# fegennari/3DWorld

Hardware: AMD Instinct MI355X
Metric: heightmap Gcells/sec (noise+erosion), 16384^2 grid (higher is better)
Workload: dtype f32

## Files before the change

### 3dworld_amd/csrc/terra_driver.hpp

```cpp
#pragma once
#include "terra_common.hpp"
#include "terra_noise.hpp"
#include "terra_erosion.hpp"
#include "terra_landscape.hpp"
#include "terra_modmap.hpp"
#include "terra_treemap.hpp"
#include "terra_treeplace.hpp"
#include "terra_decidplace.hpp"
#include "terra_sceneryplace.hpp"
#include "terra_flowers.hpp"
#include "terra_grassview.hpp"
#include "terra_treeao.hpp"
#include "terra_treeedit.hpp"
#include "terra_stage.hpp"
#include "../../include/terra.h"
#include <vector>
#include <map>
#include <string>
#include <algorithm>
#include <cmath>
#include <stdexcept>
#include <string.h>
#include <stdio.h>
#include <stdlib.h>

namespace terra {

struct sine_k_t {float xmdx[F_TABLE_SIZE], xconst[F_TABLE_SIZE], ymdy[F_TABLE_SIZE], yconst[F_TABLE_SIZE], yscale[F_TABLE_SIZE];};

struct grid_job_t {
	float mx0, my0, mdx, mdy;
	uint32_t nx, ny, nxp, nyp;
	int mode, shape, kstart, glaciate, use_sine_mag;
	float sine_offset;
	int plain_only;
	int fused = 0;
	float fast_amax = 0.0f;
	uint32_t row0 = 0;
	uint32_t ty0 = 0, tyn = 0;
};
TERRA_HD uint32_t job_window_first(grid_job_t const &job) {return job.tyn ? job.ty0*128u : 0u;}
TERRA_HD uint32_t job_window_end(grid_job_t const &job) {uint64_t const e = ((uint64_t)job.ty0 + job.tyn)*128u; return (job.tyn && e < job.ny) ? (uint32_t)e : job.ny;}
constexpr uint32_t SG_TURN_ROWS = 2048;
struct noise_turn_t {void *wait_for = nullptr, *record = nullptr; uint32_t rows = 0;};

constexpr unsigned VOX_SINES = 60, VOX_PARAMS = 7;

inline uint32_t round_up(uint32_t v, uint32_t m) {return (v + m - 1)/m*m;}

struct tile_ref_pod_t {int32_t tx, ty; uint32_t xi, yi;};
struct tile_band_t {uint32_t twx, twy, ostride, xsplit, xgap, ysplit, ygap;};
TERRA_HD uint32_t tile_band_coord(uint32_t c, uint32_t split, uint32_t gap) {return c + ((c >= split) ? gap : 0u);}

TERRA_HD float sine_cell(grid_job_t const &job, float const *xt, float const *yt, unsigned x, unsigned y) {
	float z = 0.0f;
	for (int k = job.kstart; k < F_TABLE_SIZE; ++k) {z += xt[(size_t)k*job.nxp + x]*yt[(size_t)k*job.nyp + y];}
	return z;
}
TERRA_HD float finish_cell(float z, grid_job_t const &job, noise_consts_t const &nc, sin_lut_t const &L, float const *smx, float const *smy, unsigned x, unsigned y) {
	if (job.mode == MGEN_SINE) {z = apply_noise_shape_final(z, job.shape, nc.hp);}
	if (job.glaciate) {
		float const xg = ((float)x*job.mdx + job.mx0)*nc.DX_VAL_INV, yg = ((float)(y + job.row0)*job.mdy + job.my0)*nc.DY_VAL_INV;
		z = glaciate_epilogue(z, job.use_sine_mag ? smx[x] : 0.0f, job.use_sine_mag ? smy[y] : 0.0f, job.sine_offset, xg, yg, nc, L);
	}
	return z;
}
TERRA_HD float sine_cell_fused(grid_job_t const &job, float const *xt, float const *yt, unsigned x, unsigned y) {
	float z = 0.0f;
	for (int k = job.kstart; k < F_TABLE_SIZE; ++k) {z = fmaf(xt[(size_t)k*job.nxp + x], yt[(size_t)k*job.nyp + y], z);}
	return z;
}
TERRA_HD float finish_cell_fused(float z, grid_job_t const &job, noise_consts_t const &nc, float const *smx, float const *smy, unsigned x, unsigned y) {
	if (job.glaciate) {
		if (nc.glaciate) {float const relh = (z + nc.zmax_est)*nc.zmax_est2_inv; z = fmaf((relh*relh)*relh, nc.zmax_est2, -nc.zmax_est);}
		if (job.use_sine_mag) {z = z + fmaf(smx[x], smy[y], job.sine_offset);}
	}
	return z;
}
TERRA_HD float noise_cell(grid_job_t const &job, noise_consts_t const &nc, unsigned x, unsigned y) {
	float const xval = ((float)x*job.mdx + job.mx0)*nc.DX_VAL_INV, yval = ((float)(y + job.row0)*job.mdy + job.my0)*nc.DY_VAL_INV;
	switch (job.mode) {
	case MGEN_PERLIN:      return noise_zval<MGEN_PERLIN>(xval, yval, job.shape, nc);
	case MGEN_DWARP_GPU:   return noise_zval<MGEN_DWARP_GPU>(xval, yval, job.shape, nc);
	case MGEN_SIMPLEX_GPU: return noise_zval<MGEN_SIMPLEX_GPU>(xval, yval, job.shape, nc);
	default:               return noise_zval<MGEN_SIMPLEX>(xval, yval, job.shape, nc);
	}
}


struct shadow_consts_t {
	float X_SCENE_SIZE, Y_SCENE_SIZE, DX_VAL, DY_VAL, DX_VAL_INV, DY_VAL_INV, zmin, zmax, dist, dirx, diry, dirz;
	int xsize, ysize;
	uint32_t mask_fill;
	TERRA_HD int xpos(float xval) const {return (int)((double)((xval + X_SCENE_SIZE)*DX_VAL_INV) + 0.5);}
	TERRA_HD int ypos(float yval) const {return (int)((double)((yval + Y_SCENE_SIZE)*DY_VAL_INV) + 0.5);}
	TERRA_HD float xval(int xp) const {return -X_SCENE_SIZE + DX_VAL*(float)xp;}
	TERRA_HD float yval(int yp) const {return -Y_SCENE_SIZE + DY_VAL*(float)yp;}
// ... 676 lines not shown
			sk.yscale[k] = mesh_scale_z_inv*sinTable[k][0];
			sk.xconst[k] = ms2*sinTable[k][4] + sinTable[k][2] + x_mult*mx0;
			sk.yconst[k] = ms2*sinTable[k][3] + sinTable[k][1] + y_mult*my0;
			sk.xmdx[k] = x_mult*dx; sk.ymdy[k] = y_mult*dy;
		}
		return sk;
	}

	bool sine_plain_only(int shp, int kstart) const {
		if (shp != 0 || hp.crack_lo < hp.crack_hi || (hp.volcano_width > 0.0f && hp.volcano_height > 0.0f) || consts().custom_glaciate_exp != 0.0f) return false;
		double bound = 0.0;
		for (int k = kstart; k < F_TABLE_SIZE; ++k) {bound += std::fabs((double)(mesh_scale_z_inv*sinTable[k][0]));}
		return (double)min_std(hp.plat_bot, hp.crat_h) > bound*1.001 + 1e-3;
	}

	void gen_grid_dev(float x0, float y0, float dx, float dy, uint32_t nx, uint32_t ny, uint32_t flags, int min_start_sin, float *d_out, float *h_minmax = nullptr, uint32_t row0 = 0, uint32_t nrows = 0xFFFFFFFFu, float *d_minmax = nullptr, noise_turn_t const *turn = nullptr) {
		require_scene();
		if (nx == 0 || ny == 0) throw std::invalid_argument("build_arrays: nx, ny must be > 0");
		if (nrows == 0xFFFFFFFFu) {if (row0 != 0) throw std::invalid_argument("gen_grid rows: row0 without a row count"); nrows = ny;}
		if (nrows == 0 || row0 >= ny || nrows > ny - row0) throw std::invalid_argument("gen_grid rows: [row0, row0 + nrows) must be a non-empty range inside the grid");
		grid_job_t job;
		job.mx0 = dx*x0; job.my0 = dy*y0; job.mdx = dx; job.mdy = dy; job.nx = nx; job.ny = nrows; job.row0 = row0; ny = nrows;
		job.nxp = round_up(nx, 128); job.nyp = round_up(ny, 128);
		bool const force_sine = (flags & TERRA_GEN_FORCE_SINE) != 0;
		job.mode = force_sine ? (int)MGEN_SINE : mode; job.shape = force_sine ? 0 : shape;
		job.kstart = imax(start_eval_sin, min_start_sin);
		job.glaciate = (flags & TERRA_GEN_GLACIATE) ? 1 : 0;
		job.use_sine_mag = (job.glaciate && hp.sine_mag > 0.0f) ? 1 : 0;
		job.sine_offset = hp.sine_bias*mesh_scale_z_inv;
		job.plain_only = (job.mode == MGEN_SINE && sine_plain_only(job.shape, job.kstart)) ? 1 : 0;
		job.fused = (((flags & (TERRA_GEN_FUSED | TERRA_GEN_FAST)) || opt.gen_fused) && fused_kernel_exists(job.mode, job.plain_only != 0)) ? (((flags & TERRA_GEN_FAST) || opt.gen_fused == 2) ? 2 : 1) : 0;
		job.fast_amax = sine_amp_max(job.kstart);
		noise_consts_t const nc = consts();
		sin_lut_t const L = lut();
		float *smx = scratch<float>(s_smx, job.nxp), *smy = scratch<float>(s_smy, job.nyp);
		uint32_t *d_mm = nullptr;
		bool const sine = (job.mode == MGEN_SINE);
		if (turn && turn->wait_for) {BE::event_synchronize(turn->wait_for);}
		if (h_minmax || d_minmax || sine) {d_mm = scratch<uint32_t>(s_mm, 2); if (!sine) {be.fill32(d_mm, 0xFFFFFFFFu, 2);}}
		bool fused;
		bool const sm_on = job.use_sine_mag != 0;
		float const sm_scale = hp.sine_mag*mesh_scale_z_inv, sm_freq = mesh_scale*hp.sine_freq, dxi = DX_VAL_INV, dyi = DY_VAL_INV;
		if (sm_on && job.mode != MGEN_SINE) {
			float const mx0 = job.mx0, my0 = job.my0, mdx = dx, mdy = dy;
			uint32_t const nxp = job.nxp, nyp = job.nyp;
			be.launch((size_t)nxp + nyp, [=] TERRA_LAMBDA (size_t i) {
				if (i < nxp) {smx[i] = (i < nx) ? sm_scale*L.COSF(((float)(unsigned)i*mdx + mx0)*dxi*sm_freq) : 0.0f;}
				else {unsigned const y = (unsigned)(i - nxp); smy[y] = (y < ny) ? L.COSF(((float)(y + row0)*mdy + my0)*dyi*sm_freq) : 0.0f;}
			});
		}
		if (job.mode == MGEN_SINE) {
			float const *st = sinTable_dev();
			float const msx = mesh_scale*DX_VAL_INV, msy = mesh_scale*DY_VAL_INV, ms2 = (float)(0.5*(double)mesh_scale), mszi = mesh_scale_z_inv, jmx0 = job.mx0, jmy0 = job.my0, mdx = dx, mdy = dy;
			float *xt = scratch<float>(s_xt, (size_t)F_TABLE_SIZE*job.nxp), *yt = scratch<float>(s_yt, (size_t)F_TABLE_SIZE*job.nyp);
			uint32_t const nxp = job.nxp, nyp = job.nyp;
			size_t const ntab = (size_t)F_TABLE_SIZE*(nxp + nyp);
			uint32_t *const mmz = d_mm;
			be.launch(ntab + (sm_on ? (size_t)nxp + nyp : 0), [=] TERRA_LAMBDA (size_t i) {
				if (i == 0) {mmz[0] = 0xFFFFFFFFu; mmz[1] = 0xFFFFFFFFu;}
				if (i < (size_t)F_TABLE_SIZE*nxp) {
					unsigned const k = (unsigned)(i / nxp), x = (unsigned)(i % nxp);
					float const *stk = st + 5*k;
					float const x_mult = msx*stk[4], xconst = ms2*stk[4] + stk[2] + x_mult*jmx0, xmdx = x_mult*mdx;
					xt[i] = (x < nx) ? L.SINF(xmdx*(float)x + xconst) : 0.0f;
				}
				else if (i < ntab) {
					size_t const j = i - (size_t)F_TABLE_SIZE*nxp;
					unsigned const k = (unsigned)(j / nyp), y = (unsigned)(j % nyp);
					float const *stk = st + 5*k;
					float const y_mult = msy*stk[3], yscale = mszi*stk[0], yconst = ms2*stk[3] + stk[1] + y_mult*jmy0, ymdy = y_mult*mdy;
					yt[j] = (y < ny) ? yscale*L.SINF(ymdy*(float)(y + row0) + yconst) : 0.0f;
				}
				else {
					size_t const q = i - ntab;
					if (q < nxp) {smx[q] = (q < nx) ? sm_scale*L.COSF(((float)(unsigned)q*mdx + jmx0)*dxi*sm_freq) : 0.0f;}
					else {unsigned const y = (unsigned)(q - nxp); smy[y] = (y < ny) ? L.COSF(((float)(y + row0)*mdy + jmy0)*dyi*sm_freq) : 0.0f;}
				}
			});
			uint32_t *const mm_arg = (h_minmax || d_minmax) ? d_mm : nullptr;
			uint32_t const nty = (ny + 127u)/128u, tail = (turn && turn->record && !job.fused) ? std::min((turn->rows + 127u)/128u, nty) : 0u;
			if (tail > 0 && tail < nty) {
				grid_job_t part = job;
				part.ty0 = 0; part.tyn = nty - tail;
				fused = be.sine_grid(part, nc, L, xt, yt, smx, smy, d_out, mm_arg);
				be.event_record(turn->record);
				part.ty0 = nty - tail; part.tyn = tail;
				be.sine_grid(part, nc, L, xt, yt, smx, smy, d_out, mm_arg);
			}
			else {
				fused = be.sine_grid(job, nc, L, xt, yt, smx, smy, d_out, mm_arg);
				if (turn && turn->record) {be.event_record(turn->record);}
			}
		}
		else {
			fused = be.noise_grid(job, nc, L, smx, smy, d_out, (h_minmax || d_minmax) ? d_mm : nullptr, d_noise_lut);
			if (turn && turn->record) {be.event_record(turn->record);}
		}
		if ((h_minmax || d_minmax) && !fused) {be.minmax(d_out, (size_t)nx*ny, d_mm);}
		if (d_minmax) {uint32_t const *mm = d_mm; be.launch(1, [=] TERRA_LAMBDA (size_t) {d_minmax[0] = ord2f(mm[0]); d_minmax[1] = ord2f(~mm[1]);}, 64);}
		if (h_minmax) {
			uint32_t out[2];
			be.d2h(out, d_mm, sizeof(out));
			h_minmax[0] = ord2f(out[0]); h_minmax[1] = ord2f(~out[1]);
		}
	}

	float eval_mesh_sin_terms(float xv, float yv) const {
		require_scene();
		sin_lut_t const HL = host_lut();
		float zval = 0.0f;
		for (int k = start_eval_sin; k < F_TABLE_SIZE; ++k) {
			float const *stk = sinTable[k];
			zval += stk[0]*HL.SINF(stk[3]*yv + stk[1])*HL.SINF(stk[4]*xv + stk[2]);
		}
		return zval;
	}
	void eval_points_dev(float const *d_xy, uint32_t n, uint32_t kind, float xy_scale, int no_xyoff, int xoff2, int yoff2, float *d_out) {
		require_scene();
		if (n == 0) return;
		if (kind > 1) throw std::invalid_argument("eval_points: kind must be TERRA_POINTS_SCALED or TERRA_POINTS_EXACT");
		noise_consts_t const nc = consts();
		sin_lut_t const L = lut();
		float const *st = sinTable_dev();
		hmap_view_t const hv = hmap_view();
		bool const hm = using_hmap(), hm_detail = using_hmap_with_detail();
		int const md = mode, shp = shape, k0 = start_eval_sin;
// ... 530 lines not shown
		report.window_shifts = hc.n_shift;
		report.critical_steps = hc.crit_steps; report.critical_shifts = hc.crit_shifts;
		report.clk_wave = hc.clk_wave; report.clk_init = hc.clk_init; report.clk_shift = hc.clk_shift; report.clk_tail = hc.clk_tail; report.clk_critical = hc.clk_crit;
		report.clk_shift_flush = hc.clk_sh_flush; report.clk_shift_prep = hc.clk_sh_prep; report.clk_shift_load = hc.clk_sh_load;
		report.crit_clk_flush = hc.crit_own_flush; report.crit_clk_load = hc.crit_own_load; report.crit_clk_prep = hc.crit_own_prep;
		report.crit_clk_shift = hc.crit_own_shift; report.crit_clk_edge = hc.crit_own_edge; report.crit_steps_own = hc.crit_own_steps;
		if (!record_touched) return false;
		uint32_t const ntouched = hc.touched;
		if (ntouched > sb.touched_cap) return false;
		uint32_t const *tch = sb.touched; float const mz = ec.min_zval; grid_view_t const gg = g;
		be.launch(ntouched, [=] TERRA_LAMBDA (size_t i) {touched_clamp_body(gg, tch, (uint32_t)i, d_min ? *d_min : mz);});
		return true;
	}

	uint32_t tile_size() const {return (uint32_t)cfg.mesh_x;}
	void require_tile_size() const {
		int const S = cfg.mesh_x;
		if (S == 128) return;
		if (S < 16 || S > 1024) throw std::invalid_argument("tiles: the tile size (mesh_x) must be 16 .. 1024");
		if (cfg.mesh_y != S) throw std::invalid_argument("tiles: at a tile size other than 128 mesh_x and mesh_y must be equal (the reference asserts it in tiled mode)");
		if ((S & 3) == 2) throw std::invalid_argument("tiles: a tile size of the form 4k + 2 is not supported (the reference's sub-block loop would read row and column S + 2, past the zvals)");
	}
	void require_tile_128(char const *what) const {
		if (cfg.mesh_x != 128) throw std::invalid_argument(std::string(what) + ": only at the tile size 128 (mesh_x = 128)");
	}
	tile_ref_pod_t const *tile_fields_dev(int32_t const *tile_xy, uint32_t n, uint32_t tw, int shift, float *d_out, float xy_scale = 1.0f,
		bool glac = true, bool force_sine = false, int min_start_sin = 0,
		tile_band_t const *band = nullptr, bool *band_used = nullptr,
		float y_scale = 0.0f)
	{
		uint32_t const size = tile_size(), zv = tw;
		if (band_used) {*band_used = false;}
		float const fdx = xy_scale*DX_VAL, fdy = ((y_scale != 0.0f) ? y_scale : xy_scale)*DY_VAL;
		std::vector<int32_t> ux, uy;
		for (uint32_t i = 0; i < n; ++i) {ux.push_back(tile_xy[2*i]); uy.push_back(tile_xy[2*i+1]);}
		std::sort(ux.begin(), ux.end()); ux.erase(std::unique(ux.begin(), ux.end()), ux.end());
		std::sort(uy.begin(), uy.end()); uy.erase(std::unique(uy.begin(), uy.end()), uy.end());
		typedef tile_ref_pod_t tile_ref_t;
		std::vector<tile_ref_t> refs(n);
		for (uint32_t i = 0; i < n; ++i) {
			refs[i].tx = tile_xy[2*i]; refs[i].ty = tile_xy[2*i+1];
			refs[i].xi = (uint32_t)(std::lower_bound(ux.begin(), ux.end(), refs[i].tx) - ux.begin());
			refs[i].yi = (uint32_t)(std::lower_bound(uy.begin(), uy.end(), refs[i].ty) - uy.begin());
		}
		uint32_t const nux = (uint32_t)ux.size(), nuy = (uint32_t)uy.size();
		bool unique_tiles = true;
		{std::vector<std::pair<int32_t, int32_t>> tt; for (uint32_t i = 0; i < n; ++i) {tt.push_back(std::make_pair(tile_xy[2*i], tile_xy[2*i+1]));} std::sort(tt.begin(), tt.end()); unique_tiles = (std::adjacent_find(tt.begin(), tt.end()) == tt.end());}
		int const md_ = force_sine ? (int)MGEN_SINE : mode;
		bool const banded = band && xy_scale != 0.0f && d_out && be.tile_band_ok(n, nux, nuy, band->twx, unique_tiles, md_ == MGEN_SINE && sine_plain_only(force_sine ? 0 : shape, imax(start_eval_sin, min_start_sin)), md_);
		if (band_used) {*band_used = banded;}
		tile_band_t const bd = banded ? *band : tile_band_t{zv, zv, zv, 0xFFFFFFFFu, 0u, 0xFFFFFFFFu, 0u};
		uint32_t const zvx = bd.twx, zvy = bd.twy;
		uint32_t const nxpv = round_up(nux*zvx, 128), nypv = round_up(nuy*zvy, 128);
		size_t const tab_floats = (size_t)F_TABLE_SIZE*(nxpv + nypv), sm_floats = (size_t)nux*zvx + (size_t)nuy*zvy;
		stage_layout_t par_lay;
		size_t const o_refs = par_lay.add_bytes(refs.size()*sizeof(tile_ref_t)), o_m0 = par_lay.add_bytes((size_t)(nux + nuy)*4), o_sk = par_lay.add_bytes((nux + nuy)*sizeof(sine_k_t));
		size_t const par_bytes = par_lay.total;
		size_t const bytes = par_bytes + (tab_floats + sm_floats)*4 + 1024;
		uint8_t *base = scratch<uint8_t>(s_tiles, bytes);
		tile_ref_t *d_refs = (tile_ref_t *)(base + o_refs);
		float *d_m0 = (float *)(base + o_m0);
		sine_k_t *d_sk = (sine_k_t *)(base + o_sk);
		float *d_tab = (float *)(base + par_bytes);
		float *d_sm = d_tab + tab_floats;
		std::vector<uint8_t> par((xy_scale == 0.0f) ? o_m0 : par_bytes, 0);
		memcpy(par.data() + o_refs, refs.data(), refs.size()*sizeof(tile_ref_t));
		if (xy_scale == 0.0f) {be.h2d_async(base, par.data(), par.size()); return d_refs;}
		{
			float *h_m0 = (float *)(par.data() + o_m0); sine_k_t *sks = (sine_k_t *)(par.data() + o_sk);
			for (uint32_t i = 0; i < nux; ++i) {float const x0 = (float)((ux[i]*(int)size - shift) - cfg.mesh_x/2); h_m0[i] = fdx*x0; sks[i] = make_sine_k(h_m0[i], 0.0f, fdx, fdy);}
			for (uint32_t i = 0; i < nuy; ++i) {float const y0 = (float)((uy[i]*(int)size - shift) - cfg.mesh_y/2); h_m0[nux+i] = fdy*y0; sks[nux+i] = make_sine_k(0.0f, h_m0[nux+i], fdx, fdy);}
		}
		be.h2d_async(base, par.data(), par.size());
		noise_consts_t const nc = consts();
		sin_lut_t const L = lut();
		int const md = force_sine ? (int)MGEN_SINE : mode, shp = force_sine ? 0 : shape, kstart = imax(start_eval_sin, min_start_sin);
		bool const use_sm = glac && (hp.sine_mag > 0.0f);
		float const dxv = fdx, dyv = fdy, dxi = DX_VAL_INV, dyi = DY_VAL_INV;
		if (use_sm) {
			float const sm_scale = hp.sine_mag*mesh_scale_z_inv, freq = mesh_scale*hp.sine_freq;
			size_t const nsx = (size_t)nux*zvx;
			be.launch(sm_floats, [=] TERRA_LAMBDA (size_t i) {
				if (i < nsx) {unsigned const u = (unsigned)(i / zvx), c = tile_band_coord((unsigned)(i % zvx), bd.xsplit, bd.xgap); d_sm[i] = sm_scale*L.COSF(((float)c*dxv + d_m0[u])*dxi*freq);}
				else {size_t const j = i - nsx; unsigned const u = (unsigned)(j / zvy), c = tile_band_coord((unsigned)(j % zvy), bd.ysplit, bd.ygap); d_sm[i] = L.COSF(((float)c*dyv + d_m0[nux + u])*dyi*freq);}
			});
		}
		float *d_taby = d_tab + (size_t)F_TABLE_SIZE*nxpv;
		if (md == MGEN_SINE) {
			be.launch(tab_floats, [=] TERRA_LAMBDA (size_t i) {
				bool const isx = i < (size_t)F_TABLE_SIZE*nxpv;
				size_t const j = isx ? i : i - (size_t)F_TABLE_SIZE*nxpv;
				unsigned const rowlen = isx ? nxpv : nypv, per = isx ? zvx : zvy, k = (unsigned)(j / rowlen), v = (unsigned)(j % rowlen), u = v / per;
				unsigned const c = isx ? tile_band_coord(v % per, bd.xsplit, bd.xgap) : tile_band_coord(v % per, bd.ysplit, bd.ygap);
				float val = 0.0f;
				if (u < (isx ? nux : nuy)) {
					sine_k_t const &sk = d_sk[isx ? u : nux + u];
					val = isx ? L.SINF(sk.xmdx[k]*(float)c + sk.xconst[k]) : sk.yscale[k]*L.SINF(sk.ymdy[k]*(float)c + sk.yconst[k]);
				}
				d_tab[i] = val;
			});
		}
		float const sine_offset = hp.sine_bias*mesh_scale_z_inv;
		bool const plain = md == MGEN_SINE && sine_plain_only(shp, kstart);
		be.tile_grid(n, d_refs, nux, nuy, d_tab, d_taby, nxpv, nypv, d_sm, d_m0, md, shp, kstart, use_sm, sine_offset, nc, L, dxv, dyv, d_out, plain, banded ? zvx : tw, unique_tiles, glac, d_noise_lut, fused_kernel_exists(md, plain) ? opt.gen_fused : 0, sine_amp_max(kstart),
			banded ? &bd : nullptr);
		return d_refs;
	}

	static constexpr uint32_t AO_DIRS = 8, AO_STEPS = 8, AO_RAY_LEN = AO_STEPS*(AO_STEPS + 1)/2, AO_CTX = 129 + 2*AO_RAY_LEN;
	uint32_t ao_ctx_size() const {return tile_size() + 1 + 2*AO_RAY_LEN;}
	bool ao_context_zvals() const {return tiled_mesh_ao && mode >= MGEN_SIMPLEX_GPU;}

	bool using_hmap() const {return hmap_pix != nullptr;}
	bool using_hmap_with_detail() const {return using_hmap() && mesh_scale < 0.75f;}
	hmap_view_t hmap_view() const {return hmap_view_t{hmap_pix, hmap_w, hmap_h, hmap_nc, mesh_scale, mesh_height_scale, mesh_file_scale, mesh_file_tz, mesh_scale_z_inv};}
	void set_mesh_height_scales_for_zval_range(float min_z, float dz) {
		if (!(dz > 0.0f)) throw std::invalid_argument("set_mesh_height_scales_for_zval_range: dz must be > 0");
		float const READ_MESH_H_SCALE = 0.0008f;
		mesh_file_scale = dz/(READ_MESH_H_SCALE*mesh_height_scale*mesh_scale_z_inv);
		mesh_file_tz    = min_z/mesh_scale_z_inv;
	}
	tile_ref_pod_t const *tile_hmap_fields_dev(int32_t const *tile_xy, uint32_t n, uint32_t tw, int shift, float *d_out) {
		bool const add_detail = using_hmap_with_detail();
		tile_ref_pod_t const *d_refs = tile_fields_dev(tile_xy, n, tw, shift, d_out, add_detail ? 16.0f : 0.0f);
		hmap_view_t const hv = hmap_view();
		int const S = (int)tile_size();
		be.launch((size_t)n*tw*tw, [=] TERRA_LAMBDA (size_t i) {
			unsigned const t = (unsigned)(i / ((size_t)tw*tw)), p = (unsigned)(i % ((size_t)tw*tw)), y = p / tw, x = p % tw;
			tile_ref_pod_t const r = d_refs[t];
			float zval = hv.clamped_height(r.tx*S - shift + (int)x, r.ty*S - shift + (int)y);
			if (add_detail) {zval += 0.01f*d_out[i];}
			d_out[i] = zval;
		});
		return d_refs;
	}

	void tiles_create_zvals_dev(int32_t const *tile_xy, uint32_t n, uint32_t iters_tt, float *d_zvals, terra_tile_stats *d_stats, uint8_t *d_normals, float *d_min_nz) {
		require_scene();
		require_tile_size();
		if (n == 0) return;
		uint32_t const size = tile_size(), zv = size + 2;
		tile_ref_pod_t const *d_refs;
		if (using_hmap()) {d_refs = tile_hmap_fields_dev(tile_xy, n, zv, 0, d_zvals); iters_tt = 0;}
		else if (ao_context_zvals()) {
			uint32_t const cs = ao_ctx_size(), rl = AO_RAY_LEN;
			float *d_ctx = scratch<float>(s_ao, (size_t)n*cs*cs);
			d_refs = tile_fields_dev(tile_xy, n, cs, (int)AO_RAY_LEN, d_ctx);
			be.launch((size_t)n*zv*zv, [=] TERRA_LAMBDA (size_t i) {
				unsigned const t = (unsigned)(i / (zv*zv)), p = (unsigned)(i % (zv*zv)), y = p / zv, x = p % zv;
				d_zvals[i] = d_ctx[(size_t)t*cs*cs + (size_t)(y + rl)*cs + (x + rl)];
			});
		}
// ... 1317 lines not shown
```

### 3dworld_amd/csrc/terra_kernels.hpp

```cpp
#pragma once
#include "terra_driver.hpp"
#include "terra_noise_kernels.hpp"

namespace terra {

typedef float    st_f4 __attribute__((ext_vector_type(4)));
typedef uint32_t st_u4 __attribute__((ext_vector_type(4)));

template<class F> __global__ void k_generic(size_t n, F f) {
	size_t const i = (size_t)blockIdx.x*blockDim.x + threadIdx.x;
	if (i < n) {f(i);}
}

template<class F> __global__ __launch_bounds__(64) void k_waves(F f, unsigned first) {
	__builtin_amdgcn_s_setprio(3);
	__shared__ __attribute__((aligned(16))) float win[EW*EW];
	__shared__ uint8_t dirty[EW*EW];
	__shared__ wave_shared_t sh;
	wave_scratch_t const ws{win, dirty, &sh};
	f((size_t)blockIdx.x + first, ws);
}

template<class F> __global__ __launch_bounds__(64) void k_waves_nolds(F f) {f((size_t)blockIdx.x);}

template<class F> __global__ __launch_bounds__(64) __attribute__((amdgpu_waves_per_eu(4))) void k_waves_lean(F f) {
	__builtin_amdgcn_s_setprio(3);
	__shared__ __attribute__((aligned(16))) float win[EW*EW];
	__shared__ uint8_t dirty[EW*EW];
	__shared__ lean_shared_t sh;
	lean_scratch_t const ws{win, dirty, &sh};
	f((size_t)blockIdx.x, ws);
}


constexpr int SG_BX = 128, SG_BY = 128, SG_TX = 8, SG_TY = 8, SG_THREADS = 256, SG_KC = 45;
__device__ __forceinline__ bool sg_tile_of_block(unsigned b, unsigned ntx, unsigned nty, unsigned rowgroup, unsigned &bx, unsigned &by) {
	unsigned const nb = ntx*nty, per_xcd = (nb + 7)/8;
	unsigned const lin = (b & 7)*per_xcd + (b >> 3);
	if (lin >= nb) return false;
	unsigned const group = lin/(rowgroup*ntx), r = lin % (rowgroup*ntx);
	unsigned const rows_here = (nty - group*rowgroup < rowgroup) ? nty - group*rowgroup : rowgroup;
	bx = r/rows_here; by = group*rowgroup + r % rows_here;
	return bx < ntx;
}

struct sg_tiles_t {int32_t const *tile_map; float const *m0; uint32_t nux; uint32_t rowgroup; uint32_t tw;
	uint32_t twy, ostride, xsplit, xgap, ysplit, ygap;};

typedef float sg_v2f __attribute__((ext_vector_type(2)));
__device__ __forceinline__ void sg_mul_add_2x8(sg_v2f (&r0)[SG_TX/2], sg_v2f (&r1)[SG_TX/2], sg_v2f const (&xp)[4], sg_v2f yp) {
	sg_v2f t0, t1;
#define TERRA_SG_2X2(A0, A1, X) \
	"v_pk_mul_f32 %8, " X ", %13 op_sel:[0,0] op_sel_hi:[1,0]\n\t" \
	"v_pk_mul_f32 %9, " X ", %13 op_sel:[0,1] op_sel_hi:[1,1]\n\t" \
	"v_pk_add_f32 " A0 ", " A0 ", %8\n\t" \
	"v_pk_add_f32 " A1 ", " A1 ", %9\n\t"
	asm(TERRA_SG_2X2("%0", "%4", "%10") TERRA_SG_2X2("%1", "%5", "%11") TERRA_SG_2X2("%2", "%6", "%12") TERRA_SG_2X2("%3", "%7", "%14")
	    : "+v"(r0[0]), "+v"(r0[1]), "+v"(r0[2]), "+v"(r0[3]), "+v"(r1[0]), "+v"(r1[1]), "+v"(r1[2]), "+v"(r1[3]), "=&v"(t0), "=&v"(t1)
	    : "v"(xp[0]), "v"(xp[1]), "v"(xp[2]), "v"(yp), "v"(xp[3]));
#undef TERRA_SG_2X2
}
struct sg_xop_t {float4 a, b;};
__device__ __forceinline__ sg_xop_t sg_load_x(float const *px, int k) {return sg_xop_t{*(float4 const *)(px + k*SG_BX), *(float4 const *)(px + k*SG_BX + 64)};}
__device__ __forceinline__ void sg_accumulate_half(sg_v2f (&acc)[SG_TY][SG_TX/2], sg_xop_t const &x, float4 const &y, int h) {
	sg_v2f const xp[4] = {{x.a.x, x.a.y}, {x.a.z, x.a.w}, {x.b.x, x.b.y}, {x.b.z, x.b.w}};
	sg_mul_add_2x8(acc[4*h], acc[4*h + 1], xp, sg_v2f{y.x, y.y});
	sg_mul_add_2x8(acc[4*h + 2], acc[4*h + 3], xp, sg_v2f{y.z, y.w});
}

template<bool TILES, bool GENERAL, int KC = SG_KC> __global__ __launch_bounds__(SG_THREADS) void k_sine_grid(grid_job_t job, noise_consts_t nc, sin_lut_t L,
	float const *__restrict__ xt, float const *__restrict__ yt, float const *__restrict__ smx, float const *__restrict__ smy, float *__restrict__ out, unsigned ntx, unsigned nty, uint32_t *__restrict__ mm, sg_tiles_t tiles)
{
	__shared__ __attribute__((aligned(16))) float sX[(KC + 2)*SG_BX];
	__shared__ __attribute__((aligned(16))) float sY[(KC + 2)*SG_BY];
	unsigned bxi, byi;
	if (!sg_tile_of_block(blockIdx.x, ntx, nty, tiles.rowgroup, bxi, byi)) return;
	if (!TILES) {byi += job.ty0;}
	uint32_t mm_lo = 0xFFFFFFFFu, mm_hi = 0xFFFFFFFFu;
	unsigned const tid = threadIdx.x, bx0 = bxi*SG_BX, by0 = byi*SG_BY;
	unsigned const tx = tid & 15, ty = tid >> 4;
	float const *px = sX + tx*4, *py = sY + ty*4;
	sg_v2f acc[SG_TY][SG_TX/2];
#pragma unroll
	for (int i = 0; i < SG_TY; ++i) {
#pragma unroll
		for (int jp = 0; jp < SG_TX/2; ++jp) {acc[i][jp] = sg_v2f{0.0f, 0.0f};}
	}
	int const nk = F_TABLE_SIZE - job.kstart, nchunks = (nk + KC - 1)/KC, per_chunk = (nk + nchunks - 1)/nchunks;
	for (int c = 0; c < nchunks; ++c) {
		int const k0 = job.kstart + c*per_chunk, kn = ((k0 + per_chunk > F_TABLE_SIZE) ? F_TABLE_SIZE - k0 : per_chunk);
		if (c > 0) {__syncthreads();}
		{
			constexpr int ITERS = (KC*(SG_BX/4) + SG_THREADS - 1)/SG_THREADS;
			unsigned const kr = tid >> 5, q4 = (tid & 31u)*4u;
			float const *const gx = xt + (size_t)(k0 + (int)kr)*job.nxp + bx0 + q4, *const gy = yt + (size_t)(k0 + (int)kr)*job.nyp + by0 + q4;
#pragma unroll
			for (int tab = 0; tab < 2; ++tab) {
				float const *const g = tab ? gy : gx; size_t const stride = tab ? job.nyp : job.nxp; float *const sT = tab ? sY : sX;
				float4 v[ITERS];
#pragma unroll
				for (int it = 0; it < ITERS; ++it) {v[it] = make_float4(0.0f, 0.0f, 0.0f, 0.0f); if ((int)kr + 8*it < kn) {v[it] = *(float4 const *)(g + (size_t)(8*it)*stride);}}
#pragma unroll
				for (int it = 0; it < ITERS; ++it) {if ((int)kr + 8*it < kn) {*(float4 *)&sT[(kr + 8u*it)*SG_BX + q4] = v[it];}}
			}
		}
		__syncthreads();
		sg_xop_t XA = sg_load_x(px, 0), XB = sg_load_x(px, 1);
		float4 ya = *(float4 const *)py, yb = *(float4 const *)(py + 64);
		int k = 0;
		for (; k + 1 < kn; k += 2) {
			sg_accumulate_half(acc, XA, ya, 0); __builtin_amdgcn_sched_barrier(0); ya = *(float4 const *)(py + (k + 1)*SG_BY);
			sg_accumulate_half(acc, XA, yb, 1); __builtin_amdgcn_sched_barrier(0); yb = *(float4 const *)(py + (k + 1)*SG_BY + 64); XA = sg_load_x(px, k + 2);
			sg_accumulate_half(acc, XB, ya, 0); __builtin_amdgcn_sched_barrier(0); ya = *(float4 const *)(py + (k + 2)*SG_BY);
			sg_accumulate_half(acc, XB, yb, 1); __builtin_amdgcn_sched_barrier(0); yb = *(float4 const *)(py + (k + 2)*SG_BY + 64); XB = sg_load_x(px, k + 3);
		}
		if (k < kn) {sg_accumulate_half(acc, XA, ya, 0); sg_accumulate_half(acc, XA, yb, 1);}
	}
	bool const vec_ok = ((job.nx & 3u) == 0) && !TILES;
	if (!GENERAL && TILES && (job.nx & 3u) == 0) {
		typedef sg_v2f v2f;
		typedef float st_f4u __attribute__((ext_vector_type(4), aligned(4)));
		bool const gl = job.glaciate && nc.glaciate, sm = job.glaciate && job.use_sine_mag;
		float4 sx[2], sy[2];
		sx[0] = sx[1] = sy[0] = sy[1] = make_float4(0.0f, 0.0f, 0.0f, 0.0f);
		if (sm) {
#pragma unroll
			for (int h = 0; h < 2; ++h) {
				unsigned const x = bx0 + h*64 + tx*4, y = by0 + h*64 + ty*4;
				if (x < job.nx) {sx[h] = *(float4 const *)(smx + x);}
				sy[h] = make_float4((y < job.ny) ? smy[y] : 0.0f, (y + 1 < job.ny) ? smy[y + 1] : 0.0f, (y + 2 < job.ny) ? smy[y + 2] : 0.0f, (y + 3 < job.ny) ? smy[y + 3] : 0.0f);
			}
		}
		v2f const zme = {nc.zmax_est, nc.zmax_est}, inv = {nc.zmax_est2_inv, nc.zmax_est2_inv}, z2 = {nc.zmax_est2, nc.zmax_est2}, off = {job.sine_offset, job.sine_offset};
		unsigned const tw = tiles.tw, twy = tiles.twy, os = tiles.ostride, nuy = job.ny/twy;
		unsigned ux0[2], cx0[2], uy0[2], cy0[2];
#pragma unroll
		for (int half = 0; half < 2; ++half) {unsigned const x = bx0 + half*64 + tx*4; ux0[half] = x/tw; cx0[half] = x - ux0[half]*tw;}
#pragma unroll
		for (int g = 0; g < 2; ++g) {unsigned const y = by0 + g*64 + ty*4; uy0[g] = y/twy; cy0[g] = y - uy0[g]*twy;}
		int tmap[2][2][2][2];
#pragma unroll
		for (int g = 0; g < 2; ++g) {
#pragma unroll
			for (int dy = 0; dy < 2; ++dy) {
#pragma unroll
				for (int half = 0; half < 2; ++half) {
#pragma unroll
					for (int dx = 0; dx < 2; ++dx) {
						unsigned const uy = uy0[g] + dy, ux = ux0[half] + dx;
						tmap[g][dy][half][dx] = (uy < nuy && ux < tiles.nux) ? tiles.tile_map[uy*tiles.nux + ux] : -1;
					}
				}
			}
		}
#pragma unroll
		for (int i = 0; i < SG_TY; ++i) {
			unsigned const y = by0 + (i >> 2)*64 + ty*4 + (i & 3);
			if (y >= job.ny) continue;
			float const syq[4] = {sy[i >> 2].x, sy[i >> 2].y, sy[i >> 2].z, sy[i >> 2].w};
			v2f const syi = {syq[i & 3], syq[i & 3]};
			unsigned cy = cy0[i >> 2] + (unsigned)(i & 3); int dy = 0;
			if (cy >= twy) {cy -= twy; dy = 1;}
			unsigned const oy = cy + ((cy >= tiles.ysplit) ? tiles.ygap : 0u);
#pragma unroll
			for (int half = 0; half < 2; ++half) {
				unsigned const x = bx0 + half*64 + tx*4;
				if (x >= job.nx) continue;
				v2f z01 = acc[i][half*2], z23 = acc[i][half*2 + 1];
				if (gl) {
					v2f const r01 = (z01 + zme)*inv, r23 = (z23 + zme)*inv;
					z01 = ((r01*r01)*r01)*z2 - zme; z23 = ((r23*r23)*r23)*z2 - zme;
				}
				if (sm) {
					v2f const s01 = {sx[half].x, sx[half].y}, s23 = {sx[half].z, sx[half].w};
					z01 = z01 + (s01*syi + off); z23 = z23 + (s23*syi + off);
				}
				unsigned const cx = cx0[half];
				int const ta = dy ? tmap[i >> 2][1][half][0] : tmap[i >> 2][0][half][0], tb = dy ? tmap[i >> 2][1][half][1] : tmap[i >> 2][0][half][1];
				if (cx + 3 < tw && (cx + 3 < tiles.xsplit || cx >= tiles.xsplit)) {
					unsigned const ox = cx + ((cx >= tiles.xsplit) ? tiles.xgap : 0u);
					if (ta >= 0) {*(st_f4u *)(out + (size_t)ta*os*os + oy*os + ox) = st_f4u{z01.x, z01.y, z23.x, z23.y};}
				}
				else {
					float const v[4] = {z01.x, z01.y, z23.x, z23.y};
#pragma unroll
					for (int j = 0; j < 4; ++j) {
						bool const next = cx + (unsigned)j >= tw;
						int const t = next ? tb : ta;
						unsigned const cxx = next ? cx + (unsigned)j - tw : cx + (unsigned)j, ox = cxx + ((cxx >= tiles.xsplit) ? tiles.xgap : 0u);
						if (t >= 0) {out[(size_t)t*os*os + oy*os + ox] = v[j];}
					}
				}
			}
		}
		return;
	}
	if (!GENERAL && !TILES && vec_ok) {
		typedef sg_v2f v2f;
		bool const gl = job.glaciate && nc.glaciate, sm = job.glaciate && job.use_sine_mag;
		float4 sx[2], sy[2];
		sx[0] = sx[1] = sy[0] = sy[1] = make_float4(0.0f, 0.0f, 0.0f, 0.0f);
		if (sm) {
			sx[0] = *(float4 const *)(smx + bx0 + tx*4); sx[1] = *(float4 const *)(smx + bx0 + 64 + tx*4);
			sy[0] = *(float4 const *)(smy + by0 + ty*4); sy[1] = *(float4 const *)(smy + by0 + 64 + ty*4);
		}
		v2f const zme = {nc.zmax_est, nc.zmax_est}, inv = {nc.zmax_est2_inv, nc.zmax_est2_inv}, z2 = {nc.zmax_est2, nc.zmax_est2}, off = {job.sine_offset, job.sine_offset};
		float fmn = INFINITY, fmx = -INFINITY;
#pragma unroll
		for (int i = 0; i < SG_TY; ++i) {
			unsigned const y = by0 + (i >> 2)*64 + ty*4 + (i & 3);
			if (y >= job.ny) continue;
			float const syq[4] = {sy[i >> 2].x, sy[i >> 2].y, sy[i >> 2].z, sy[i >> 2].w};
			v2f const syi = {syq[i & 3], syq[i & 3]};
#pragma unroll
			for (int half = 0; half < 2; ++half) {
				unsigned const x = bx0 + half*64 + tx*4;
				if (x >= job.nx) continue;
				v2f z01 = acc[i][half*2], z23 = acc[i][half*2 + 1];
				if (gl) {
					v2f const r01 = (z01 + zme)*inv, r23 = (z23 + zme)*inv;
					z01 = ((r01*r01)*r01)*z2 - zme; z23 = ((r23*r23)*r23)*z2 - zme;
				}
				if (sm) {
					v2f const s01 = {sx[half].x, sx[half].y}, s23 = {sx[half].z, sx[half].w};
					z01 = z01 + (s01*syi + off); z23 = z23 + (s23*syi + off);
				}
				fmn = sg_min3(sg_min3(fmn, z01.x, z01.y), z23.x, z23.y);
				fmx = sg_max3(sg_max3(fmx, z01.x, z01.y), z23.x, z23.y);
				*(float4 *)(out + (size_t)y*job.nx + x) = make_float4(z01.x, z01.y, z23.x, z23.y);
			}
		}
		if (mm) {
			if (fmn <= fmx) {mm_lo = f2ord(fmn); mm_hi = ~f2ord(fmx);}
			wave_minmax_publish(mm_lo, mm_hi, mm);
		}
		return;
	}
	hmap_params_t const &hp = nc.hp;
	bool const plain = !GENERAL || ((job.shape == 0) && !(hp.crack_lo < hp.crack_hi) && !(hp.volcano_width > 0.0f && hp.volcano_height > 0.0f));
	float const pp_limit = min_std(hp.plat_bot, hp.crat_h);
	float smxv[SG_TX], smyv[SG_TY];
#pragma unroll
	for (int j = 0; j < SG_TX; ++j) {unsigned const x = bx0 + (j >> 2)*64 + tx*4 + (j & 3); smxv[j] = (job.use_sine_mag && x < job.nx) ? smx[x] : 0.0f;}
#pragma unroll
	for (int i = 0; i < SG_TY; ++i) {unsigned const y = by0 + (i >> 2)*64 + ty*4 + (i & 3); smyv[i] = (job.use_sine_mag && y < job.ny) ? smy[y] : 0.0f;}
	float fmn = INFINITY, fmx = -INFINITY;
	unsigned t_ux[2] = {0, 0}, t_cx[2] = {0, 0}, t_uy[4] = {0, 0, 0, 0}, t_cy[4] = {0, 0, 0, 0};
	if (TILES) {
#pragma unroll
		for (int half = 0; half < 2; ++half) {unsigned const x = bx0 + half*64 + tx*4; t_ux[half] = x/tiles.tw; t_cx[half] = x - t_ux[half]*tiles.tw;}
#pragma unroll
		for (int g = 0; g < 4; ++g) {unsigned const y = by0 + g*64 + ty*4; t_uy[g] = y/tiles.tw; t_cy[g] = y - t_uy[g]*tiles.tw;}
	}
#pragma unroll
	for (int i = 0; i < SG_TY; ++i) {
		unsigned const y = by0 + (i >> 2)*64 + ty*4 + (i & 3);
		if (y >= job.ny) continue;
#pragma unroll
		for (int half = 0; half < 2; ++half) {
			unsigned const x = bx0 + half*64 + tx*4;
			if (x >= job.nx) continue;
			float v[4];
#pragma unroll
			for (int j = 0; j < 4; ++j) {
				float z = acc[i][half*2 + (j >> 1)][j & 1];
				if (!GENERAL || (plain && !(z > pp_limit))) {
					if (job.glaciate) {
						if (nc.glaciate) {float const relh = (z + nc.zmax_est)*nc.zmax_est2_inv; z = (GENERAL ? glaciate_exp_fn(relh, nc.custom_glaciate_exp) : relh*relh*relh)*nc.zmax_est2 - nc.zmax_est;}
						if (job.use_sine_mag) {z += smxv[half*4 + j]*smyv[i] + job.sine_offset;}
					}
				}
				else if (GENERAL && x + j < job.nx) {
					if (TILES) {
						unsigned const tw = tiles.tw, ux = (x + j)/tw, uy = y/tw;
						grid_job_t jt = job; jt.mx0 = tiles.m0[ux]; jt.my0 = tiles.m0[tiles.nux + uy];
						z = finish_cell(z, jt, nc, L, smx + ux*tw, smy + uy*tw, (x + j) - ux*tw, y - uy*tw);
					}
					else {z = finish_cell(z, job, nc, L, smx, smy, x + j, y);}
				}
				else {z = 0.0f;}
				v[j] = z;
				if (x + j < job.nx) {fmn = fminf(fmn, z); fmx = fmaxf(fmx, z);}
			}
			if (TILES) {
// ... 1836 lines not shown
```

Before: 325.1.

## Pad sine tables with zero rows to drop staging bounds checks and simplify addressing

Pads the x/y sine tables with extra zeroed rows past F_TABLE_SIZE so the LDS staging in k_sine_grid can load whole 8-row groups without per-row bounds checks, and only fills rows from kstart onward. The inner accumulation loop is unrolled by four terms, using byte-offset LDS addressing advanced with an explicit add. The epilogue gains specialised branches for full interior tiles with compile-time glaciate and sine-mag flags, which removes bounds checks and simplifies store addresses. In exchange the tables use more memory and the kernel has more code variants and inline asm to maintain.

```diff
diff --git a/3dworld_amd/csrc/terra_driver.hpp b/3dworld_amd/csrc/terra_driver.hpp
--- a/3dworld_amd/csrc/terra_driver.hpp
+++ b/3dworld_amd/csrc/terra_driver.hpp
@@ -43,6 +43,23 @@
 TERRA_HD uint32_t job_window_end(grid_job_t const &job) {uint64_t const e = ((uint64_t)job.ty0 + job.tyn)*128u; return (job.tyn && e < job.ny) ? (uint32_t)e : job.ny;}
 constexpr uint32_t SG_TURN_ROWS = 2048;
 struct noise_turn_t {void *wait_for = nullptr, *record = nullptr; uint32_t rows = 0;};
+
+constexpr int SG_KCS[3] = {20, 27, 45};
+constexpr int SG_TABLE_ROWS = F_TABLE_SIZE + 48;
+constexpr bool sg_kc_listed(int kc) {return kc == SG_KCS[0] || kc == SG_KCS[1] || kc == SG_KCS[2];}
+constexpr int sg_stage_iters(int kc) {return (kc*32 + 255)/256;}
+constexpr int sg_rows_end(int kstart, int kc) {
+	int const nk = F_TABLE_SIZE - kstart;
+	if (nk <= 0) return F_TABLE_SIZE;
+	int const nchunks = (nk + kc - 1)/kc, per_chunk = (nk + nchunks - 1)/nchunks;
+	return kstart + (nchunks - 1)*per_chunk + 8*sg_stage_iters(kc);
+}
+inline int sg_table_rows_end(int kstart) {
+	int e = F_TABLE_SIZE;
+	for (int kc : SG_KCS) {if (sg_rows_end(kstart, kc) > e) {e = sg_rows_end(kstart, kc);}}
+	if (kstart < 0 || e > SG_TABLE_ROWS) throw std::logic_error("sine tables: a chunk of k_sine_grid would read behind the rows allocated");
+	return e;
+}
 
 constexpr unsigned VOX_SINES = 60, VOX_PARAMS = 7;
 
@@ -825,26 +842,34 @@
 		if (job.mode == MGEN_SINE) {
 			float const *st = sinTable_dev();
 			float const msx = mesh_scale*DX_VAL_INV, msy = mesh_scale*DY_VAL_INV, ms2 = (float)(0.5*(double)mesh_scale), mszi = mesh_scale_z_inv, jmx0 = job.mx0, jmy0 = job.my0, mdx = dx, mdy = dy;
-			float *xt = scratch<float>(s_xt, (size_t)F_TABLE_SIZE*job.nxp), *yt = scratch<float>(s_yt, (size_t)F_TABLE_SIZE*job.nyp);
-			uint32_t const nxp = job.nxp, nyp = job.nyp;
-			size_t const ntab = (size_t)F_TABLE_SIZE*(nxp + nyp);
+			float *xt = scratch<float>(s_xt, (size_t)SG_TABLE_ROWS*job.nxp), *yt = scratch<float>(s_yt, (size_t)SG_TABLE_ROWS*job.nyp);
+			uint32_t const nxp = job.nxp, nyp = job.nyp, kfirst = (uint32_t)imin(job.kstart, F_TABLE_SIZE), nrw = (uint32_t)sg_table_rows_end((int)kfirst) - kfirst;
+			size_t const nxtab = (size_t)nrw*nxp, ntab = (size_t)nrw*((size_t)nxp + nyp), nall = ntab + (sm_on ? (size_t)nxp + nyp : 0);
 			uint32_t *const mmz = d_mm;
-			be.launch(ntab + (sm_on ? (size_t)nxp + nyp : 0), [=] TERRA_LAMBDA (size_t i) {
+			be.launch(nall ? nall : 1, [=] TERRA_LAMBDA (size_t i) {
 				if (i == 0) {mmz[0] = 0xFFFFFFFFu; mmz[1] = 0xFFFFFFFFu;}
-				if (i < (size_t)F_TABLE_SIZE*nxp) {
-					unsigned const k = (unsigned)(i / nxp), x = (unsigned)(i % nxp);
-					float const *stk = st + 5*k;
-					float const x_mult = msx*stk[4], xconst = ms2*stk[4] + stk[2] + x_mult*jmx0, xmdx = x_mult*mdx;
-					xt[i] = (x < nx) ? L.SINF(xmdx*(float)x + xconst) : 0.0f;
+				if (i < nxtab) {
+					unsigned const k = kfirst + (unsigned)(i / nxp), x = (unsigned)(i % nxp);
+					float v = 0.0f;
+					if (k < (unsigned)F_TABLE_SIZE && x < nx) {
+						float const *stk = st + 5*k;
+						float const x_mult = msx*stk[4], xconst = ms2*stk[4] + stk[2] + x_mult*jmx0, xmdx = x_mult*mdx;
+						v = L.SINF(xmdx*(float)x + xconst);
+					}
+					xt[(size_t)kfirst*nxp + i] = v;
 				}
 				else if (i < ntab) {
-					size_t const j = i - (size_t)F_TABLE_SIZE*nxp;
-					unsigned const k = (unsigned)(j / nyp), y = (unsigned)(j % nyp);
-					float const *stk = st + 5*k;
-					float const y_mult = msy*stk[3], yscale = mszi*stk[0], yconst = ms2*stk[3] + stk[1] + y_mult*jmy0, ymdy = y_mult*mdy;
-					yt[j] = (y < ny) ? yscale*L.SINF(ymdy*(float)(y + row0) + yconst) : 0.0f;
-				}
-				else {
+					size_t const j = i - nxtab;
+					unsigned const k = kfirst + (unsigned)(j / nyp), y = (unsigned)(j % nyp);
+					float v = 0.0f;
+					if (k < (unsigned)F_TABLE_SIZE && y < ny) {
+						float const *stk = st + 5*k;
+						float const y_mult = msy*stk[3], yscale = mszi*stk[0], yconst = ms2*stk[3] + stk[1] + y_mult*jmy0, ymdy = y_mult*mdy;
+						v = yscale*L.SINF(ymdy*(float)(y + row0) + yconst);
+					}
+					yt[(size_t)kfirst*nyp + j] = v;
+				}
+				else if (i < nall) {
 					size_t const q = i - ntab;
 					if (q < nxp) {smx[q] = (q < nx) ? sm_scale*L.COSF(((float)(unsigned)q*mdx + jmx0)*dxi*sm_freq) : 0.0f;}
 					else {unsigned const y = (unsigned)(q - nxp); smy[y] = (y < ny) ? L.COSF(((float)(y + row0)*mdy + jmy0)*dyi*sm_freq) : 0.0f;}
@@ -1481,7 +1506,8 @@
 		tile_band_t const bd = banded ? *band : tile_band_t{zv, zv, zv, 0xFFFFFFFFu, 0u, 0xFFFFFFFFu, 0u};
 		uint32_t const zvx = bd.twx, zvy = bd.twy;
 		uint32_t const nxpv = round_up(nux*zvx, 128), nypv = round_up(nuy*zvy, 128);
-		size_t const tab_floats = (size_t)F_TABLE_SIZE*(nxpv + nypv), sm_floats = (size_t)nux*zvx + (size_t)nuy*zvy;
+		uint32_t const kfirst = (uint32_t)imin(imax(start_eval_sin, min_start_sin), F_TABLE_SIZE), trows = (uint32_t)sg_table_rows_end((int)kfirst);
+		size_t const tab_floats = (size_t)trows*(nxpv + nypv), sm_floats = (size_t)nux*zvx + (size_t)nuy*zvy;
 		stage_layout_t par_lay;
 		size_t const o_refs = par_lay.add_bytes(refs.size()*sizeof(tile_ref_t)), o_m0 = par_lay.add_bytes((size_t)(nux + nuy)*4), o_sk = par_lay.add_bytes((nux + nuy)*sizeof(sine_k_t));
 		size_t const par_bytes = par_lay.total;
@@ -1514,19 +1540,20 @@
 				else {size_t const j = i - nsx; unsigned const u = (unsigned)(j / zvy), c = tile_band_coord((unsigned)(j % zvy), bd.ysplit, bd.ygap); d_sm[i] = L.COSF(((float)c*dyv + d_m0[nux + u])*dyi*freq);}
 			});
 		}
-		float *d_taby = d_tab + (size_t)F_TABLE_SIZE*nxpv;
+		float *d_taby = d_tab + (size_t)trows*nxpv;
 		if (md == MGEN_SINE) {
-			be.launch(tab_floats, [=] TERRA_LAMBDA (size_t i) {
-				bool const isx = i < (size_t)F_TABLE_SIZE*nxpv;
-				size_t const j = isx ? i : i - (size_t)F_TABLE_SIZE*nxpv;
-				unsigned const rowlen = isx ? nxpv : nypv, per = isx ? zvx : zvy, k = (unsigned)(j / rowlen), v = (unsigned)(j % rowlen), u = v / per;
+			size_t const nxtab = (size_t)(trows - kfirst)*nxpv;
+			be.launch((size_t)(trows - kfirst)*(nxpv + nypv), [=] TERRA_LAMBDA (size_t i) {
+				bool const isx = i < nxtab;
+				size_t const j = isx ? i : i - nxtab;
+				unsigned const rowlen = isx ? nxpv : nypv, per = isx ? zvx : zvy, k = kfirst + (unsigned)(j / rowlen), v = (unsigned)(j % rowlen), u = v / per;
 				unsigned const c = isx ? tile_band_coord(v % per, bd.xsplit, bd.xgap) : tile_band_coord(v % per, bd.ysplit, bd.ygap);
 				float val = 0.0f;
-				if (u < (isx ? nux : nuy)) {
+				if (k < (unsigned)F_TABLE_SIZE && u < (isx ? nux : nuy)) {
 					sine_k_t const &sk = d_sk[isx ? u : nux + u];
 					val = isx ? L.SINF(sk.xmdx[k]*(float)c + sk.xconst[k]) : sk.yscale[k]*L.SINF(sk.ymdy[k]*(float)c + sk.yconst[k]);
 				}
-				d_tab[i] = val;
+				(isx ? d_tab : d_taby)[(size_t)kfirst*rowlen + j] = val;
 			});
 		}
 		float const sine_offset = hp.sine_bias*mesh_scale_z_inv;
diff --git a/3dworld_amd/csrc/terra_kernels.hpp b/3dworld_amd/csrc/terra_kernels.hpp
--- a/3dworld_amd/csrc/terra_kernels.hpp
+++ b/3dworld_amd/csrc/terra_kernels.hpp
@@ -61,7 +61,6 @@
 #undef TERRA_SG_2X2
 }
 struct sg_xop_t {float4 a, b;};
-__device__ __forceinline__ sg_xop_t sg_load_x(float const *px, int k) {return sg_xop_t{*(float4 const *)(px + k*SG_BX), *(float4 const *)(px + k*SG_BX + 64)};}
 __device__ __forceinline__ void sg_accumulate_half(sg_v2f (&acc)[SG_TY][SG_TX/2], sg_xop_t const &x, float4 const &y, int h) {
 	sg_v2f const xp[4] = {{x.a.x, x.a.y}, {x.a.z, x.a.w}, {x.b.x, x.b.y}, {x.b.z, x.b.w}};
 	sg_mul_add_2x8(acc[4*h], acc[4*h + 1], xp, sg_v2f{y.x, y.y});
@@ -79,7 +78,6 @@
 	uint32_t mm_lo = 0xFFFFFFFFu, mm_hi = 0xFFFFFFFFu;
 	unsigned const tid = threadIdx.x, bx0 = bxi*SG_BX, by0 = byi*SG_BY;
 	unsigned const tx = tid & 15, ty = tid >> 4;
-	float const *px = sX + tx*4, *py = sY + ty*4;
 	sg_v2f acc[SG_TY][SG_TX/2];
 #pragma unroll
 	for (int i = 0; i < SG_TY; ++i) {
@@ -91,7 +89,9 @@
 		int const k0 = job.kstart + c*per_chunk, kn = ((k0 + per_chunk > F_TABLE_SIZE) ? F_TABLE_SIZE - k0 : per_chunk);
 		if (c > 0) {__syncthreads();}
 		{
-			constexpr int ITERS = (KC*(SG_BX/4) + SG_THREADS - 1)/SG_THREADS;
+			constexpr int ITERS = sg_stage_iters(KC);
+			static_assert(sg_kc_listed(KC), "sg_table_rows_end() sizes the zero rows of the tables for the chunk sizes in SG_KCS");
+			static_assert(SG_BX == 128 && SG_BY == 128 && SG_THREADS == 256 && 8*ITERS >= KC && 8*(ITERS - 1) < KC + 2, "row groups of 8: every row of a chunk staged, all but the last group inside the LDS rows");
 			unsigned const kr = tid >> 5, q4 = (tid & 31u)*4u;
 			float const *const gx = xt + (size_t)(k0 + (int)kr)*job.nxp + bx0 + q4, *const gy = yt + (size_t)(k0 + (int)kr)*job.nyp + by0 + q4;
 #pragma unroll
@@ -99,21 +99,30 @@
 				float const *const g = tab ? gy : gx; size_t const stride = tab ? job.nyp : job.nxp; float *const sT = tab ? sY : sX;
 				float4 v[ITERS];
 #pragma unroll
-				for (int it = 0; it < ITERS; ++it) {v[it] = make_float4(0.0f, 0.0f, 0.0f, 0.0f); if ((int)kr + 8*it < kn) {v[it] = *(float4 const *)(g + (size_t)(8*it)*stride);}}
-#pragma unroll
-				for (int it = 0; it < ITERS; ++it) {if ((int)kr + 8*it < kn) {*(float4 *)&sT[(kr + 8u*it)*SG_BX + q4] = v[it];}}
-			}
-		}
-		__syncthreads();
-		sg_xop_t XA = sg_load_x(px, 0), XB = sg_load_x(px, 1);
-		float4 ya = *(float4 const *)py, yb = *(float4 const *)(py + 64);
+				for (int it = 0; it < ITERS; ++it) {v[it] = *(float4 const *)(g + (size_t)(8*it)*stride);}
+#pragma unroll
+				for (int it = 0; it < ITERS; ++it) {if (8*it + 8 <= KC + 2 || kr + 8u*it < (unsigned)(KC + 2)) {*(float4 *)&sT[(kr + 8u*it)*SG_BX + q4] = v[it];}}
+			}
+		}
+		__syncthreads();
+		unsigned ox = tx*16u, oy = ty*16u;
+		auto const ldx = [&](unsigned o, int row) {char const *const b = (char const *)sX + o; return sg_xop_t{*(float4 const *)(b + row*(SG_BX*4)), *(float4 const *)(b + row*(SG_BX*4) + 256)};};
+		auto const ldy = [&](unsigned o, int row, int h) {return *(float4 const *)((char const *)sY + o + row*(SG_BY*4) + h*256);};
+		sg_xop_t XA = ldx(ox, 0), XB = ldx(ox, 1);
+		float4 ya = ldy(oy, 0, 0), yb = ldy(oy, 0, 1);
+		auto const two_terms = [&](auto first) {
+			constexpr int FIRST = decltype(first)::value;
+			sg_accumulate_half(acc, XA, ya, 0); __builtin_amdgcn_sched_barrier(0); ya = ldy(oy, FIRST + 1, 0);
+			sg_accumulate_half(acc, XA, yb, 1); __builtin_amdgcn_sched_barrier(0); yb = ldy(oy, FIRST + 1, 1); XA = ldx(ox, FIRST + 2);
+			sg_accumulate_half(acc, XB, ya, 0); __builtin_amdgcn_sched_barrier(0); ya = ldy(oy, FIRST + 2, 0);
+			sg_accumulate_half(acc, XB, yb, 1); __builtin_amdgcn_sched_barrier(0); yb = ldy(oy, FIRST + 2, 1); XB = ldx(ox, FIRST + 3);
+		};
 		int k = 0;
-		for (; k + 1 < kn; k += 2) {
-			sg_accumulate_half(acc, XA, ya, 0); __builtin_amdgcn_sched_barrier(0); ya = *(float4 const *)(py + (k + 1)*SG_BY);
-			sg_accumulate_half(acc, XA, yb, 1); __builtin_amdgcn_sched_barrier(0); yb = *(float4 const *)(py + (k + 1)*SG_BY + 64); XA = sg_load_x(px, k + 2);
-			sg_accumulate_half(acc, XB, ya, 0); __builtin_amdgcn_sched_barrier(0); ya = *(float4 const *)(py + (k + 2)*SG_BY);
-			sg_accumulate_half(acc, XB, yb, 1); __builtin_amdgcn_sched_barrier(0); yb = *(float4 const *)(py + (k + 2)*SG_BY + 64); XB = sg_load_x(px, k + 3);
-		}
+		for (; k + 3 < kn; k += 4) {
+			two_terms(std::integral_constant<int, 0>()); two_terms(std::integral_constant<int, 2>());
+			asm volatile("v_add_u32 %0, %2, %0\n\tv_add_u32 %1, %2, %1" : "+v"(ox), "+v"(oy) : "s"(4u*SG_BX*4u));
+		}
+		if (k + 1 < kn) {two_terms(std::integral_constant<int, 0>()); k += 2;}
 		if (k < kn) {sg_accumulate_half(acc, XA, ya, 0); sg_accumulate_half(acc, XA, yb, 1);}
 	}
 	bool const vec_ok = ((job.nx & 3u) == 0) && !TILES;
@@ -197,39 +206,53 @@
 	}
 	if (!GENERAL && !TILES && vec_ok) {
 		typedef sg_v2f v2f;
-		bool const gl = job.glaciate && nc.glaciate, sm = job.glaciate && job.use_sine_mag;
+		bool const gl_rt = job.glaciate && nc.glaciate, sm_rt = job.glaciate && job.use_sine_mag;
 		float4 sx[2], sy[2];
 		sx[0] = sx[1] = sy[0] = sy[1] = make_float4(0.0f, 0.0f, 0.0f, 0.0f);
-		if (sm) {
+		if (sm_rt) {
 			sx[0] = *(float4 const *)(smx + bx0 + tx*4); sx[1] = *(float4 const *)(smx + bx0 + 64 + tx*4);
 			sy[0] = *(float4 const *)(smy + by0 + ty*4); sy[1] = *(float4 const *)(smy + by0 + 64 + ty*4);
 		}
 		v2f const zme = {nc.zmax_est, nc.zmax_est}, inv = {nc.zmax_est2_inv, nc.zmax_est2_inv}, z2 = {nc.zmax_est2, nc.zmax_est2}, off = {job.sine_offset, job.sine_offset};
 		float fmn = INFINITY, fmx = -INFINITY;
-#pragma unroll
-		for (int i = 0; i < SG_TY; ++i) {
-			unsigned const y = by0 + (i >> 2)*64 + ty*4 + (i & 3);
-			if (y >= job.ny) continue;
-			float const syq[4] = {sy[i >> 2].x, sy[i >> 2].y, sy[i >> 2].z, sy[i >> 2].w};
-			v2f const syi = {syq[i & 3], syq[i & 3]};
-#pragma unroll
-			for (int half = 0; half < 2; ++half) {
-				unsigned const x = bx0 + half*64 + tx*4;
-				if (x >= job.nx) continue;
-				v2f z01 = acc[i][half*2], z23 = acc[i][half*2 + 1];
-				if (gl) {
-					v2f const r01 = (z01 + zme)*inv, r23 = (z23 + zme)*inv;
-					z01 = ((r01*r01)*r01)*z2 - zme; z23 = ((r23*r23)*r23)*z2 - zme;
+		auto const rows = [&](auto inside, auto gl_in, auto sm_in) {
+			constexpr bool INSIDE = decltype(inside)::value;
+			bool const gl = INSIDE ? decltype(gl_in)::value : gl_rt, sm = INSIDE ? decltype(sm_in)::value : sm_rt;
+			char *const obase = (char *)(out + ((size_t)by0*job.nx + bx0));
+			unsigned const voff = ((ty*4u)*job.nx + tx*4u)*4u;
+#pragma unroll
+			for (int i = 0; i < SG_TY; ++i) {
+				unsigned const y = by0 + (i >> 2)*64 + ty*4 + (i & 3);
+				if (!INSIDE && y >= job.ny) continue;
+				float const syq[4] = {sy[i >> 2].x, sy[i >> 2].y, sy[i >> 2].z, sy[i >> 2].w};
+				v2f const syi = {syq[i & 3], syq[i & 3]};
+#pragma unroll
+				for (int half = 0; half < 2; ++half) {
+					unsigned const x = bx0 + half*64 + tx*4;
+					if (!INSIDE && x >= job.nx) continue;
+					v2f z01 = acc[i][half*2], z23 = acc[i][half*2 + 1];
+					if (gl) {
+						v2f const r01 = (z01 + zme)*inv, r23 = (z23 + zme)*inv;
+						z01 = ((r01*r01)*r01)*z2 - zme; z23 = ((r23*r23)*r23)*z2 - zme;
+					}
+					if (sm) {
+						v2f const s01 = {sx[half].x, sx[half].y}, s23 = {sx[half].z, sx[half].w};
+						z01 = z01 + (s01*syi + off); z23 = z23 + (s23*syi + off);
+					}
+					fmn = sg_min3(sg_min3(fmn, z01.x, z01.y), z23.x, z23.y);
+					fmx = sg_max3(sg_max3(fmx, z01.x, z01.y), z23.x, z23.y);
+					char *const orow = obase + (size_t)((i >> 2)*64 + (i & 3))*job.nx*4u + half*256;
+					float4 *const o = INSIDE ? (float4 *)(orow + voff) : (float4 *)(out + (size_t)y*job.nx + x);
+					*o = make_float4(z01.x, z01.y, z23.x, z23.y);
 				}
-				if (sm) {
-					v2f const s01 = {sx[half].x, sx[half].y}, s23 = {sx[half].z, sx[half].w};
-					z01 = z01 + (s01*syi + off); z23 = z23 + (s23*syi + off);
-				}
-				fmn = sg_min3(sg_min3(fmn, z01.x, z01.y), z23.x, z23.y);
-				fmx = sg_max3(sg_max3(fmx, z01.x, z01.y), z23.x, z23.y);
-				*(float4 *)(out + (size_t)y*job.nx + x) = make_float4(z01.x, z01.y, z23.x, z23.y);
-			}
-		}
+			}
+		};
+		std::true_type const T{}; std::false_type const F{};
+		if (bx0 + SG_BX <= job.nx && by0 + SG_BY <= job.ny && job.nx <= (1u << 24)) {
+			if (gl_rt) {if (sm_rt) {rows(T, T, T);} else {rows(T, T, F);}}
+			else       {if (sm_rt) {rows(T, F, T);} else {rows(T, F, F);}}
+		}
+		else {rows(F, F, F);}
 		if (mm) {
 			if (fmn <= fmx) {mm_lo = f2ord(fmn); mm_hi = ~f2ord(fmx);}
 			wave_minmax_publish(mm_lo, mm_hi, mm);
```

New measurement: 319.1. -1.8%, worse.
